# RichardZJM/lammps-mtp-kokkos

Hardware: AMD Instinct MI355X
Metric: atom-steps/s (64k-atom W, level-16 MTP) (higher is better)
Workload: dtype f64; 1 GPU; 65536-atom BCC W (a=3.165 A, +-0.05 A jitter, seed 777), W_L16.mtp (B=130 T=894 S=116 A=332 R=8 Mu=4 C=149), rc=5 A, full list 7 A, eflag=1 vflag=1; atoms=65536, potential=W_L16.mtp, parallelism=single GPU, atoms_rank0=65536, list_entries_rank0=5802796

## Files before the change

lammps_mtp_kokkos_amd/csrc/mtp_context.hip:

```cpp
#include <hip/hip_runtime.h>

#include <unistd.h>

#include <algorithm>
#include <cerrno>
#include <cmath>
#include <cstdio>
#include <cstdlib>
#include <cstring>
#include <new>
#include <string>
#include <vector>

#include "../../include/mtp_mi355x.h"
#include "mtp_device.hpp"
#include "mtp_shape_fields.hpp"
#include "mtp_potential.hpp"

namespace {

struct HipFail {
  hipError_t e;
  const char *what;
};
// ... 391 lines not shown
  bb.off_pack = put(pot.basic_pack_lds.data(), pot.basic_pack_lds.size() * sizeof(int32_t));
  blob.resize((blob.size() + 15) / 16 * 16, 0);
  bs.norows = (int) blob.size();
  bb.off_rows = put(rows8.data(), rows8.size() * sizeof(MtpRow8));
  bb.off_leaf_cf = put(pot.leaf_cf.data(), pot.leaf_cf.size() * sizeof(double));
  bb.off_leaf_cb = pot.leaf_cb == pot.leaf_cf ? bb.off_leaf_cf : put(pot.leaf_cb.data(), pot.leaf_cb.size() * sizeof(double));
  blob.resize((blob.size() + 15) / 16 * 16, 0);
  bs.rows = (int) blob.size();
  bb.blob_bytes = bs.norows;
  bb.rows_in_lds = 0;
}

void fill_sizes(const mtp_potential &pot, MtpDevParams &b)
{
  b.Sp = pot.species_count;
  b.R = pot.radial_basis_size;
  b.Mu = pot.radial_func_count;
  b.P = pot.max_alpha_index_basic;
  b.A = pot.alpha_moment_count;
  b.B = pot.alpha_index_basic_count;
  b.T = pot.alpha_index_times_count;
  b.S = pot.alpha_scalar_count;
  b.C = pot.coeff_count;
  b.nslot = pot.slot_count;
  b.coef_total = pot.coef_total;
  b.coef_dense = pot.coef_dense;
  for (int d = 0; d <= MTP_PSTRIDE; d++) {
    b.deg_first[d] = pot.deg_first[d];
    b.deg_coef[d] = pot.deg_coef[d];
  }
  b.nlevels = pot.normal_levels;
  const bool lv_fit = pot.level_offset.size() == (size_t) pot.normal_levels + 2 && pot.level_offset.size() <= MTP_SHAPE_ARR_LEN;
  for (int k = 0; k < MTP_SHAPE_ARR_LEN; k++) b.level_rows[k] = lv_fit && k < (int) pot.level_offset.size() ? pot.level_offset[k] : 0;
  b.nseed = (int) pot.seed_idx.size();
  b.Ad = pot.stored_moment_count;
  b.Am = b.Ad;
  b.Se = (int) pot.e_map.size();
}

void pad_and_tile(const double *W, int C, int cpad, std::vector<double> &pad, std::vector<double> &tiled)
{
  pad.assign((size_t) cpad * cpad, 0.0);
  for (int r = 0; r < C; r++) std::memcpy(&pad[(size_t) r * cpad], &W[(size_t) r * C], (size_t) C * sizeof(double));
  tiled.assign((size_t) cpad * cpad, 0.0);
  const int ks_n = cpad / 4;
  for (int t = 0; t < cpad / 16; t++)
    for (int ks = 0; ks < ks_n; ks++)
      for (int l = 0; l < 64; l++)
        tiled[((size_t) t * ks_n + ks) * 64 + l] = pad[(size_t) (16 * t + (l & 15)) * cpad + 4 * ks + (l >> 4)];
}

double cfg_grade_of(const double *W, int C, const double *c)
{
  double mx = 0.0;
  for (int i = 0; i < C; i++) {
    const double *row = &W[(size_t) i * C];
    double g = 0.0;
    for (int j = 0; j < C; j++) g += c[j] * row[j];
    mx = std::max(mx, g < 0 ? -g : g);
  }
  return mx;
}

bool all_finite(const double *v, size_t n)
{
  for (size_t i = 0; v && i < n; i++)
// ... 1698 lines not shown
}

extern "C" {

int mtp_plan_fixed_fields(const mtp_potential *pot, int num_cus, int inum, int max_numneigh, int variant, int grade,
                          char *buf, int buflen)
{
  MtpDevParams p;
  int rc = plan_params(pot, num_cus, inum, max_numneigh, variant, grade, p);
  if (rc != MTP_OK) return rc;
  if (!buf || buflen <= 0) return MTP_ERR_ARG;
  int KL = 0, NB = 0;
  (void) mtp_pick_fwd_shape(p.nfb, &KL, &NB);
  const int dlow = mtp_wave_kernel_deg(KL, p.P) == mtp_wave_kernel_dlow(KL);
  std::string s;
  auto put = [&](const char *k, int v) { s += std::string(k) + "=" + std::to_string(v) + "\n"; };
  put("KL", KL);
  put("NB", NB);
  put("PITCH", MTP_PITCH);
  put("GRADE", grade ? 1 : 0);
  put("DEG", mtp_wave_kernel_deg(KL, p.P));
  put("WPS", dlow && p.wps == 3 ? 3 : 2);
#define MTP_X(f) put(#f, p.f);
  MTP_SHAPE_INT_FIELDS(MTP_X)
#undef MTP_X
#define MTP_X(f)                                                                          \
  {                                                                                       \
    s += #f "=";                                                                          \
    for (int k = 0; k < MTP_SHAPE_ARR_LEN; k++) s += (k ? "," : "") + std::to_string(p.f[k]); \
    s += "\n";                                                                            \
  }
  MTP_SHAPE_ARR_FIELDS(MTP_X)
#undef MTP_X
  if ((int) s.size() + 1 > buflen) return MTP_ERR_LIMIT;
  std::memcpy(buf, s.c_str(), s.size() + 1);
  return MTP_OK;
}

int mtp_plan_fixed_shape(const mtp_potential *pot, int num_cus, int inum, int max_numneigh, int variant, int grade,
                         char *name, int namelen)
{
  MtpDevParams p;
  int rc = plan_params(pot, num_cus, inum, max_numneigh, variant, grade, p);
  if (rc != MTP_OK) return rc;
  if (!name || namelen <= 0) return MTP_ERR_ARG;
  const char *m = mtp_fixed_shape_match(p);
  std::snprintf(name, (size_t) namelen, "%s", m ? m : "");
  return MTP_OK;
}

int mtp_context_last_shape(const mtp_context *c, char *name, int namelen)
{
  if (!c || !name || namelen <= 0) return MTP_ERR_ARG;
  std::snprintf(name, (size_t) namelen, "%s", c->last_shape);
  return MTP_OK;
}

}

void *mtp_internal_resolve_stream(mtp_context *c, void *stream)
{
  return stream ? stream : (c ? reinterpret_cast<void *>(c->stream) : nullptr);
}

int mtp_internal_finish_unpack(mtp_context *c, void *stream, int eflag, int vflag, double *d_ev, double *d_f, const int *d_idx,
                               const double *d_frecv, int n3)
// ... 49 lines not shown
```

lammps_mtp_kokkos_amd/csrc/mtp_device.hpp:

```cpp
#pragma once

#include <hip/hip_runtime.h>

#include <cstddef>
#include <cstdint>

#define MTP_EV_SLOTS 4096
#define MTP_MAX_WPB 12
#define MTP_PITCH 33
#define MTP_PSTRIDE 12

struct alignas(8) MtpRow8 {
  uint32_t lo, hi;
};

struct MtpDevParams {
  int Sp, R, Mu, P, A, B, T, S, C;
  int nslot, nlevels, nseed;
  int Am, Ad, Se;
  const double *leaf_cf, *leaf_cb;
  const int *g_map_all;
  int deg_first[MTP_PSTRIDE + 2], deg_coef[MTP_PSTRIDE + 2];
  int level_rows[MTP_PSTRIDE + 2];
  int coef_total;
  int coef_dense;
  double rmin, rmax, scaling, cutsq, inv_span;
  double inv_rmax;
  const unsigned char *blob;
  int blob_bytes;
  int off_rows;
  int off_level;
  int off_slot;
  int off_radial;
  int off_seed_idx;
  int off_seed_val;
  int off_map;
  int off_lin;
  int off_pack;
  int off_fwd;
  int nfb;
  int off_smu;
  int off_coef;
  int off_leaf_cf, off_leaf_cb;
// ... 11 lines not shown
  const int *ilist, *first, *neigh;
  const double *x;
  const int *type;
  double *f;
  long long *fq;
  double *eatom;
  double *vatom;
  double *ev_slots;
  double *cvec;
  int cpad;
  double *dbasic;
  int dpad;
  int *err_flag;
  unsigned long long *stamps;
  int eflag, vflag, grade_flag;
  int xcd_map;
  int grade_fused;
  int NT;
  int tab_rows;
  int dg_mode;
  int fp_row;
  int rebuild_tables;
  int pow_row;
  int dg_off;
  int w_m, w_d, w_coef, w_nb;
  int wps;
  int row0;
  int ov_doubles;
  int cj_cap;
  int wave_doubles;
  int m_doubles;
  int d_doubles;
  float inv_mu;
};

int mtp_pick_shape(int B, int *KL, int *KB);
int mtp_pick_fwd_shape(int nblk, int *KL, int *NB);
constexpr int mtp_wave_kernel_dlow(int KL) { return KL <= 32 ? 6 : 8; }
constexpr int mtp_wave_kernel_deg(int KL, int P) { return P - 1 <= mtp_wave_kernel_dlow(KL) ? mtp_wave_kernel_dlow(KL) : 11; }
hipError_t mtp_launch_wave_kernel(const MtpDevParams &p, int grid, int wpb, size_t lds, hipStream_t st,
                                  const char **used = nullptr);
bool mtp_wave_kernel_has_wps3(int nfb, int P);
hipError_t mtp_launch_ev_finish(double *ev_slots, double *ev, hipStream_t st);
hipError_t mtp_launch_ev_finish_unpack(double *ev_slots, double *ev, int fold, double *f, const int *idx, const double *frecv,
                                       int n3, hipStream_t st);
struct mtp_context;
int mtp_internal_finish_unpack(mtp_context *c, void *stream, int eflag, int vflag, double *d_ev, double *d_f, const int *d_idx,
                               const double *d_frecv, int n3);
void *mtp_internal_resolve_stream(mtp_context *c, void *stream);
hipError_t mtp_launch_fixed_to_force(long long *fq, double *f, int nall, hipStream_t st);
hipError_t mtp_launch_zero(double *p, size_t n, hipStream_t st);
const char *mtp_kernel_build_flags();
hipError_t mtp_launch_cvec_kernel(const MtpDevParams &p, int grid, int wpb, size_t lds, hipStream_t st);
hipError_t mtp_launch_grade_kernel(const double *cvec, const double *ainv_pad, const double *ainv_tiled, int cpad,
                                   int C, int inum, const int *ilist, double *grades, double *max_grade, hipStream_t st);
hipError_t mtp_launch_colsum_kernel(const double *cvec, int cpad, int C, int inum, double *coeff_ders, hipStream_t st);
#define MTP_BATCH_BLOCK 256
#define MTP_BATCH_WAVE_ROWS 256
hipError_t mtp_launch_batch_reduce(int ncfg, const int *cfg_first, const double *eatom, const double *vatom, const double *grades,
                                   double *energy, double *virial, double *cfg_grade, hipStream_t st);
hipError_t mtp_launch_batch_colsum(const double *cvec, int cpad, int ncfg, const int *cfg_first, double *csum, int *ident,
                                   hipStream_t st);
hipError_t mtp_launch_batch_grade_scale(int ncfg, const int *cfg_first, double *cfg_grade, hipStream_t st);
const char *mtp_maxvol_build_flags();
size_t mtp_maxvol_arena_doubles(int num_cus, int C, long long N, int max_swaps);
hipError_t mtp_maxvol_run(hipStream_t st, int num_cus, double *arena, int C, const double *S, const double *W,
                          const double *d_rows, long long N, int ld, double threshold, int max_swaps, int refresh, double *S_out,
// ... 58 lines not shown
```

lammps_mtp_kokkos_amd/csrc/mtp_fixed_shapes.hpp:

```cpp
#pragma once

struct Shape_w16_force_3ps {
  static constexpr const char *name = "w16_force_3ps";
  static constexpr int kKL = 32;
  static constexpr int kNB = 1;
  static constexpr int kPITCH = 33;
  static constexpr bool kGRADE = false;
  static constexpr int kDEG = 6;
  static constexpr int kWPS = 3;
  static constexpr int Sp = 1;
  static constexpr int R = 8;
  static constexpr int Mu = 4;
  static constexpr int P = 7;
  static constexpr int A = 332;
  static constexpr int B = 130;
  static constexpr int T = 894;
  static constexpr int S = 116;
  static constexpr int C = 149;
  static constexpr int nslot = 16;
  static constexpr int nlevels = 3;
  static constexpr int nseed = 46;
  static constexpr int Am = 262;
  static constexpr int Ad = 262;
  static constexpr int Se = 46;
// ... 2 lines not shown
  static constexpr int coef_dense = 1;
  static constexpr int blob_bytes = 13888;
  static constexpr int off_rows = 4160;
  static constexpr int off_level = 0;
  static constexpr int off_slot = 128;
  static constexpr int off_radial = 320;
  static constexpr int off_seed_idx = 576;
  static constexpr int off_seed_val = 768;
  static constexpr int off_map = 1136;
  static constexpr int off_lin = 1328;
  static constexpr int off_pack = 3632;
  static constexpr int off_fwd = 1760;
  static constexpr int off_smu = 1696;
  static constexpr int off_coef = 2592;
  static constexpr int off_leaf_cf = 12352;
  static constexpr int off_leaf_cb = 12352;
  static constexpr int off_seg_fwd = 32;
  static constexpr int off_seg_bwd = 80;
  static constexpr int rows_in_lds = 1;
  static constexpr int tgt_in_lds = 1;
  static constexpr int scalars_in_lds = 1;
  static constexpr int dg_mode = 1;
  static constexpr int fp_row = 24;
  static constexpr int pow_row = 16;
  static constexpr int dg_off = 0;
  static constexpr int w_m = 528;
  static constexpr int w_d = 790;
  static constexpr int w_coef = 528;
  static constexpr int w_nb = 1221;
  static constexpr int tab_rows = 53;
  static constexpr int ov_doubles = 1221;
  static constexpr int m_doubles = 262;
  static constexpr int d_doubles = 262;
  static constexpr int deg_first(int k)
  {
    constexpr int v[14] = {0, 4, 7, 10, 12, 14, 15, 16, 16, 16, 16, 16, 16, 0};
    return v[k];
  }
  static constexpr int deg_coef(int k)
  {
    constexpr int v[14] = {0, 4, 13, 40, 76, 136, 181, 244, 244, 244, 244, 244, 244, 0};
    return v[k];
  }
  static constexpr int level_rows(int k)
  {
    constexpr int v[14] = {0, 640, 768, 832, 1024, 0, 0, 0, 0, 0, 0, 0, 0, 0};
    return v[k];
  }
};

struct Shape_w16_grade_3ps {
  static constexpr const char *name = "w16_grade_3ps";
  static constexpr int kKL = 32;
  static constexpr int kNB = 1;
  static constexpr int kPITCH = 33;
  static constexpr bool kGRADE = true;
  static constexpr int kDEG = 6;
  static constexpr int kWPS = 3;
  static constexpr int Sp = 1;
  static constexpr int R = 8;
  static constexpr int Mu = 4;
  static constexpr int P = 7;
  static constexpr int A = 332;
  static constexpr int B = 130;
  static constexpr int T = 894;
  static constexpr int S = 116;
  static constexpr int C = 149;
  static constexpr int nslot = 16;
  static constexpr int nlevels = 3;
  static constexpr int nseed = 46;
  static constexpr int Am = 332;
  static constexpr int Ad = 262;
  static constexpr int Se = 46;
  static constexpr int nfb = 26;
  static constexpr int coef_total = 244;
  static constexpr int coef_dense = 1;
  static constexpr int blob_bytes = 13888;
  static constexpr int off_rows = 4160;
  static constexpr int off_level = 0;
// ... 38 lines not shown
```

lammps_mtp_kokkos_amd/csrc/mtp_kernels.hip:

```cpp
#include <hip/hip_runtime.h>

#include <type_traits>

#include "mtp_device.hpp"

#include "mtp_kernel_common.hpp"
#include "mtp_wave_body.hpp"

namespace {

template <int KL, int NB, int PITCH, bool GRADE, int DEG, int WPS>
__global__ void __launch_bounds__(WPS == 3 ? 768 : 512, WPS) mtp_wave_kernel(const MtpDevParams p_arg)
{
  (void) p_arg;
  using SH = ShapeGeneric;
#include "mtp_wave_kernel_body.hpp"
}

__global__ void __launch_bounds__(256) mtp_fixed_to_force(long long *__restrict__ fq, double *__restrict__ f, int n3)
{
  const int e = blockIdx.x * 256 + threadIdx.x;
  if (e >= n3) return;
  const long long q = fq[e];
  if (q != 0) {
// ... 596 lines not shown

const char *mtp_kernel_build_flags()
{
#define MTP_STR2(x) #x
#define MTP_STR(x) MTP_STR2(x)
  return ""
#if MTP_PU != 2
      "MTP_PU=" MTP_STR(MTP_PU) " "
#endif
#if MTP_LD != 1
      "MTP_LD=" MTP_STR(MTP_LD) " "
#endif
#if MTP_POLY_CH != 8
      "MTP_POLY_CH=" MTP_STR(MTP_POLY_CH) " "
#endif
#if MTP_POLY_ACC != 1
      "MTP_POLY_ACC=" MTP_STR(MTP_POLY_ACC) " "
#endif
#if MTP_COEF_DPP != 1
      "MTP_COEF_DPP=" MTP_STR(MTP_COEF_DPP) " "
#endif
#if MTP_LEAF_SWEEP != 1
      "MTP_LEAF_SWEEP=" MTP_STR(MTP_LEAF_SWEEP) " "
#endif
#if MTP_E_HOIST != 1
      "MTP_E_HOIST=" MTP_STR(MTP_E_HOIST) " "
#endif
#if MTP_MU_BITS != 1
      "MTP_MU_BITS=" MTP_STR(MTP_MU_BITS) " "
#endif
#if MTP_LEVEL_ARGS != 1
      "MTP_LEVEL_ARGS=" MTP_STR(MTP_LEVEL_ARGS) " "
#endif

#if MTP_GRADE_TPB != 512 || MTP_GRADE_WPE != 2
      "MTP_GRADE_TPB=" MTP_STR(MTP_GRADE_TPB) " "
#endif
      ;
}

hipError_t mtp_launch_zero(double *p, size_t n, hipStream_t st)
{
  if (n == 0) return hipSuccess;
  const size_t n2 = n / 2;
  hipLaunchKernelGGL(mtp_zero_kernel, dim3((unsigned) ((std::max<size_t>(n2, 1) + 255) / 256)), dim3(256), 0, st,
                     reinterpret_cast<double2 *>(p), n2, p + 2 * n2, (int) (n - 2 * n2));
  return hipGetLastError();
}
```

lammps_mtp_kokkos_amd/csrc/mtp_shape_fields.hpp:

```cpp
#pragma once

#include <type_traits>

#include "mtp_device.hpp"

#define MTP_SHAPE_INT_FIELDS(X)                                                                                       \
  X(Sp) X(R) X(Mu) X(P) X(A) X(B) X(T) X(S) X(C) X(nslot) X(nlevels) X(nseed) X(Am) X(Ad) X(Se) X(nfb)                \
  X(coef_total) X(coef_dense) X(blob_bytes) X(off_rows) X(off_level) X(off_slot) X(off_radial) X(off_seed_idx)        \
  X(off_seed_val) X(off_map) X(off_lin) X(off_pack) X(off_fwd) X(off_smu) X(off_coef) X(off_leaf_cf) X(off_leaf_cb)   \
  X(off_seg_fwd) X(off_seg_bwd) X(rows_in_lds) X(tgt_in_lds) X(scalars_in_lds) X(dg_mode) X(fp_row) X(pow_row)        \
  X(dg_off) X(w_m) X(w_d) X(w_coef) X(w_nb) X(tab_rows) X(ov_doubles) X(m_doubles) X(d_doubles)
#define MTP_SHAPE_ARR_FIELDS(X) X(deg_first) X(deg_coef) X(level_rows)
#define MTP_SHAPE_ARR_LEN (MTP_PSTRIDE + 2)

struct ShapeGeneric {
  static constexpr const char *name = "";
};

namespace mtp_shape {

#define MTP_X(f)                                                                    \
  template <class SH, class = void> struct has_##f : std::false_type {};            \
  template <class SH> struct has_##f<SH, std::void_t<decltype(&SH::f)>> : std::true_type {};
MTP_SHAPE_INT_FIELDS(MTP_X)
MTP_SHAPE_ARR_FIELDS(MTP_X)
#undef MTP_X

template <class SH> bool matches(const MtpDevParams &p)
{
  bool ok = true;
#define MTP_X(f) \
  if constexpr (has_##f<SH>::value) ok = ok && p.f == SH::f;
  MTP_SHAPE_INT_FIELDS(MTP_X)
#undef MTP_X
#define MTP_X(f)                    \
  if constexpr (has_##f<SH>::value) \
    for (int k = 0; k < MTP_SHAPE_ARR_LEN; k++) ok = ok && p.f[k] == SH::f(k);
  MTP_SHAPE_ARR_FIELDS(MTP_X)
#undef MTP_X
  return ok;
}

}

const char *mtp_fixed_shape_match(const MtpDevParams &p);
hipError_t mtp_launch_wave_kernel_fixed(const MtpDevParams &p, int grid, int wpb, size_t lds, hipStream_t st, const char **used);
```

lammps_mtp_kokkos_amd/csrc/mtp_wave_body.hpp:

```cpp
#pragma once

#include <hip/hip_runtime.h>

#include <type_traits>

#include "mtp_device.hpp"

#include "mtp_kernel_common.hpp"
#include "mtp_shape_fields.hpp"

namespace {

#ifndef MTP_PU
#define MTP_PU 2
#endif

typedef const __attribute__((address_space(4))) MtpDevParams *KP;

namespace shape_get {
#define MTP_X(f)                                                                  \
  template <class SH> __device__ __forceinline__ int f(KP kp)                     \
  {                                                                               \
    if constexpr (mtp_shape::has_##f<SH>::value) return SH::f;                    \
    else return kp->f;                                                            \
  }
MTP_SHAPE_INT_FIELDS(MTP_X)
#undef MTP_X
#define MTP_X(f)                                                                  \
  template <class SH> __device__ __forceinline__ int f(KP kp, int k)              \
  {                                                                               \
    if constexpr (mtp_shape::has_##f<SH>::value) return SH::f(k);                 \
    else return kp->f[k];                                                         \
  }
MTP_SHAPE_ARR_FIELDS(MTP_X)
#undef MTP_X
}
#define SHF(f) (shape_get::f<SH>(kp))
#define SHA(f, k) (shape_get::f<SH>(kp, (k)))

#define MTP_FIXED_SCALE 1099511627776.0
static __device__ __forceinline__ void force_add(KP kp, size_t idx, double v)
{
  if (kp->fq) atomicAdd(reinterpret_cast<unsigned long long *>(kp->fq) + idx, (unsigned long long) __double2ll_rn(v * MTP_FIXED_SCALE));
  else unsafeAtomicAdd(&kp->f[idx], v);
}

template <int PITCH> struct WaveLds {
  static constexpr int NT = 32;
  double *M, *D, *coef, *tab, *nbx, *nby, *nbz, *nbr, *nbi;
  int *nbj, *nbjt, *cj;
  unsigned m_addr;
  __device__ __forceinline__ unsigned addr(const double *ptr) const { return m_addr + 8u * (unsigned) (ptr - M); }
  template <class SH> __device__ __forceinline__ WaveLds(double *base, unsigned base_addr, KP kp, SH)
  {
    tab = base;
    M = tab + SHF(w_m);
    D = tab + SHF(w_d);
    coef = tab + SHF(w_coef);
    nbx = tab + SHF(w_nb);
    m_addr = base_addr + 8u * (unsigned) (M - tab);
    nby = nbx + NT;
    nbz = nby + NT;
    nbr = nbz + NT;
    nbi = nbr + NT;
    nbj = reinterpret_cast<int *>(nbi + NT);
    nbjt = nbj + NT;
    cj = nbjt + NT;
  }
};

#define MTP_PARK 2
template <int PITCH, class SH>
__device__ __forceinline__ void build_tile(KP kp, const BlockTables &bt, const WaveLds<PITCH> &w,
                                           int t0, int cnt, int ntp, bool gather, bool powers, bool with_dg, bool do_park,
                                           double (&park)[MTP_PARK],
                                           double xi0, double xi1, double xi2, int i, int itype, int lane)
{
  if (gather) {
    if (lane < ntp) {
      const bool real = t0 + lane < cnt;
      const int j = real ? w.cj[t0 + lane] : i;
      double dx = 0, dy = 0, dz = 0, r = kp->rmax, inv = kp->inv_rmax;
      if (real) {
        const double *xj = row3(kp->x, j);
        dx = xj[0] - xi0;
        dy = xj[1] - xi1;
        dz = xj[2] - xi2;
        sqrt_and_inverse(dx * dx + dy * dy + dz * dz, r, inv);
      }
      w.nbx[lane] = dx;
      w.nby[lane] = dy;
      w.nbz[lane] = dz;
      w.nbr[lane] = r;
      w.nbi[lane] = inv;
      w.nbj[lane] = j;
      w.nbjt[lane] = real ? kp->type[j] - 1 : itype;
    }
    wave_fence();
  }
  const int Mu = SHF(Mu), P = SHF(P), R = SHF(R);
  const double mult = 2.0 * kp->inv_span;
  const int n = lane & 31, h = lane >> 5;
  if (n < ntp) {
    const double r = w.nbr[n], inv = w.nbi[n];
    const int jt = w.nbjt[n];
    const double d = r - kp->rmax;
    const double ksi = (2.0 * r - (kp->rmin + kp->rmax)) * kp->inv_span;
    double *col = w.tab + n;
    auto each_mu = [&](auto &&body) {
      double d0 = 0.0, d1 = 0.0;
      if (h < Mu) d0 = body(h);
      if (h + 2 < Mu) d1 = body(h + 2);
      for (int mu = h + 2 * MTP_PARK; mu < Mu; mu += 2) (void) body(mu);
      if (do_park) {
        park[0] = d0;
        park[1] = d1;
      }
    };
    if (R == 8) {
      double qv[8], ev[8];
      qv[0] = kp->scaling * (d * d);
      qv[1] = kp->scaling * (ksi * d * d);
      ev[0] = kp->scaling * 2.0 * d;
      ev[1] = kp->scaling * (mult * d * d + 2.0 * ksi * d);
#pragma unroll
      for (int ri = 2; ri < 8; ri++) {
        qv[ri] = 2.0 * ksi * qv[ri - 1] - qv[ri - 2];
        ev[ri] = 2.0 * (mult * qv[ri - 1] + ksi * ev[ri - 1]) - ev[ri - 2];
      }
      each_mu([&](int mu) {
        const int4 *sl4 = reinterpret_cast<const int4 *>(bt.slot + mu * MTP_PSTRIDE);
        const int4 sa = sl4[0], sb = sl4[1], sc = sl4[2];
        const int sv[MTP_PSTRIDE] = {sa.x, sa.y, sa.z, sa.w, sb.x, sb.y, sb.z, sb.w, sc.x, sc.y, sc.z, sc.w};
        const double2 *c2 = reinterpret_cast<const double2 *>(bt.radial + (mul24(itype * SHF(Sp) + jt, Mu) + mu) * 8);
        const double2 c01 = c2[0], c23 = c2[1], c45 = c2[2], c67 = c2[3];
        const double cc[8] = {c01.x, c01.y, c23.x, c23.y, c45.x, c45.y, c67.x, c67.y};
        double val = cc[0] * qv[0], der = cc[0] * ev[0];
#pragma unroll
        for (int ri = 1; ri < 8; ri++) {
          val = fma(cc[ri], qv[ri], val);
          der = fma(cc[ri], ev[ri], der);
        }
        double rp = 1.0;
#pragma unroll
        for (int nu = 0; nu < MTP_PSTRIDE; nu++) {
          if (nu < P) {
            const int sidx = sv[nu];
            const double g = val * rp;
            if (sidx >= 0) {
              double *gp = col + mul24(sidx, PITCH);
              *gp = g;
              if (with_dg) gp[SHF(dg_off)] = der * rp - nu * g * inv;
            }
            rp *= inv;
          }
        }
        return der;
      });
    } else {
      each_mu([&](int mu) {
        const int *sl = bt.slot + mu * MTP_PSTRIDE;
        const double *c = bt.radial + mul24(mul24(itype * SHF(Sp) + jt, Mu) + mu, R);
// ... 412 lines not shown
  constexpr int K = (C + 15) / 16;
  double c[K];
#pragma unroll
  for (int k = 0; k < K; k++) c[k] = lds_ld(coef_l, 16 * k);
  double a = 0.0;
  dpp_chunks<C, 0>(a, c, m);
  return a;
}
template <int C> constexpr bool coef_dpp = MTP_COEF_DPP && C >= 2;
template <int C> __device__ __forceinline__ double poly_sum(unsigned coef, const double *m)
{
  if constexpr (coef_dpp<C>) return poly_eval_dpp<C>(coef, m);
  else return poly_eval<C>(coef, m);
}

#ifndef MTP_MU_BITS
#define MTP_MU_BITS 1
#endif
template <bool PACKED> struct SlotMu {
  const int *smu;
  unsigned long long bits;
  template <bool NODG, bool GRADE> __device__ __forceinline__ int uniform(int s) const
  {
    if constexpr (PACKED) return (int) (bits >> (2 * s)) & 3;
    else return (NODG || GRADE) ? __builtin_amdgcn_readfirstlane(smu[s]) : 0;
  }
  template <bool NODG, bool GRADE> __device__ __forceinline__ int per_lane(int s) const
  {
    if constexpr (PACKED) return (int) (bits >> (2 * s)) & 3;
    else return (NODG || GRADE) ? smu[s] : 0;
  }
};

template <int NU, int DEG, int PITCH, bool GRADE, bool NODG, class SH, class SMU>
__device__ __forceinline__ void force_degree(KP kp, unsigned pcol, unsigned pcoef, unsigned pcoef_l, int part, double x,
                                             double y, double z, double *m, double &UA, double &VA, double &UB,
                                             double &VB, const SMU &smu, double inv, double rw, double *W)
{
  if constexpr (NU <= DEG) {
    constexpr int C = NU * (NU + 1) / 2;
    const unsigned pc = coef_dpp<C> ? pcoef_l : pcoef;
    if (NU < SHF(P)) {
      const int s0 = SHA(deg_first, NU), cnt = SHA(deg_first, NU + 1) - s0;
      const double inv_nu = 1.0 / NU;
      const unsigned dgo = 8u * (unsigned) SHF(dg_off);
      const unsigned pfp = pcol + 8u * (unsigned) (SHF(fp_row) * PITCH);
      const double rwn = rw * inv_nu;
      const double wa = GRADE ? (part ? z : x) * rwn : 0.0, wb = GRADE ? y * rwn : 0.0;
      {
        unsigned ca = pc + 8u * (unsigned) (SHA(deg_coef, NU) + part * 2 * C);
        unsigned cg = pcol + 8u * (unsigned) (s0 * PITCH);
        for (int it = 0; it < cnt; it++) {
          const int mu = smu.template uniform<NODG, GRADE>(s0 + it);
          const double g = lds_ld(cg, 0);
          const double dg = NODG ? lds_ld(pfp + 8u * (unsigned) (mu * PITCH), 0) : lds_ld(cg + dgo, 0);
          const double G = poly_sum<C>(ca, m);
          UA = fma(g, G, UA);
          VA = fma(dg * (NODG ? rwn : inv_nu), G, VA);
          if (GRADE) {
            const double val = G * wa;
            if (mu == 0) W[0] += val;
            else if (mu == 1) W[1] += val;
            else if (mu == 2) W[2] += val;
            else W[3] += val;
          }
          ca += 8u * 3 * C;
          cg += 8u * PITCH;
        }
      }
      for (int it = 0; 2 * it < cnt; it++) {
        const int si = 2 * it + part;
        const bool ok = si < cnt;
        const int sc = ok ? si : 0;
        const unsigned cb = pc + 8u * (unsigned) (SHA(deg_coef, NU) + C) + (unsigned) mul24(sc, 8 * 3 * C);
        const unsigned cg = pcol + (unsigned) mul24(s0 + sc, 8 * PITCH);
        const int mu_raw = smu.template per_lane<NODG, GRADE>(s0 + sc);
        const double g_raw = lds_ld(cg, 0);
        const double dg_raw = NODG ? lds_ld(pfp + (unsigned) mul24(mu_raw, 8 * PITCH), 0) : lds_ld(cg + dgo, 0);
        const double G = poly_sum<C>(cb, m);
        const double g = ok ? g_raw : 0.0, dg = ok ? dg_raw : 0.0;
        UB = fma(g, G, UB);
        VB = fma(dg * (NODG ? rwn : inv_nu), G, VB);
        const int mu = ok ? mu_raw : -1;
        if (GRADE) {
          const double val = G * wb;
#pragma unroll
          for (int v = 0; v < 4; v++) W[v] += mu == v ? val : 0.0;
        }
      }
      if constexpr (NU < DEG) {
        constexpr int T0 = (NU - 1) * NU / 2;
#pragma unroll
        for (int c = 0; c < NU; c++) m[C + c] = y * m[T0 + c];
        m[C + NU] = z * m[T0 + NU - 1];
#pragma unroll
        for (int i = 0; i < C; i++) m[i] *= x;
        force_degree<NU + 1, DEG, PITCH, GRADE, NODG, SH>(kp, pcol, pcoef, pcoef_l, part, x, y, z, m, UA, VA, UB, VB, smu, inv, rw * inv, W);
      }
    }
  }
}

}
```

lammps_mtp_kokkos_amd/csrc/mtp_wave_kernel_body.hpp:

```cpp
  constexpr int NT = 32;
  constexpr bool GATHER = KL == 64;
  constexpr bool NODG_CT = WPS == 3;
  constexpr int NG = 64 / KL;
  constexpr int NPG = NT / NG;
  static_assert(NT == 32, "the force phase maps lanes to (32 neighbours) x (2 halves)");

  KP kp = (KP) __builtin_amdgcn_kernarg_segment_ptr();
#ifdef MTP_STAMPS
  const unsigned long long st_entry = __builtin_amdgcn_s_memtime();
#endif
  kernarg_touch<(int) sizeof(MtpDevParams)>(kp);
  extern __shared__ double lds[];
  unsigned char *sh = reinterpret_cast<unsigned char *>(lds);
  const int lane = threadIdx.x & 63;
  const int wave = __builtin_amdgcn_readfirstlane(threadIdx.x >> 6);
  const int wpb = blockDim.x >> 6;

  int ii_beg, ii_end, ii_step;
  if (kp->xcd_map && (gridDim.x & 7) == 0) {
    const int chunk = (kp->inum + 7) >> 3, xcd = blockIdx.x & 7;
    const int nb8 = gridDim.x >> 3;
    if (chunk % (nb8 * wpb) != 0) ii_beg = kp->row0 + xcd * chunk + wave * nb8 + (blockIdx.x >> 3);
    else ii_beg = kp->row0 + xcd * chunk + (blockIdx.x >> 3) * wpb + wave;
    ii_end = kp->row0 + min(kp->inum, (xcd + 1) * chunk);
    ii_step = (gridDim.x >> 3) * wpb;
  } else {
    ii_step = gridDim.x * wpb;
    if (kp->inum % ii_step != 0) ii_beg = kp->row0 + wave * gridDim.x + blockIdx.x;
    else ii_beg = kp->row0 + blockIdx.x * wpb + wave;
    ii_end = kp->row0 + kp->inum;
  }
  int hd_i = 0, hd_b = 0, hd_e = 0;
  if (ii_beg < ii_end) {
    hd_i = kp->ilist[ii_beg];
    hd_b = kp->first[ii_beg];
    hd_e = kp->first[ii_beg + 1];
  }
  for (int o = threadIdx.x * 16; o < SHF(blob_bytes); o += blockDim.x * 16)
    *reinterpret_cast<uint4 *>(sh + o) = *reinterpret_cast<const uint4 *>(kp->blob + o);
  __syncthreads();
  BlockTables bt;
  bt.rows = reinterpret_cast<const MtpRow8 *>(sh + SHF(off_rows));
  bt.level = reinterpret_cast<const int *>(sh + SHF(off_level));
  bt.seg_fwd = reinterpret_cast<const int *>(sh + SHF(off_seg_fwd));
  bt.seg_bwd = reinterpret_cast<const int *>(sh + SHF(off_seg_bwd));
  bt.slot = reinterpret_cast<const int *>(sh + SHF(off_slot));
  bt.radial = reinterpret_cast<const double *>(sh + SHF(off_radial));
  bt.seed_idx = reinterpret_cast<const int *>(sh + SHF(off_seed_idx));
  bt.seed_val = reinterpret_cast<const double *>(sh + SHF(off_seed_val));
  bt.map = reinterpret_cast<const int *>(sh + SHF(off_map));
  bt.lin = reinterpret_cast<const double *>(sh + SHF(off_lin));
  bt.pack = reinterpret_cast<const int *>(sh + SHF(off_pack));
  bt.coef = reinterpret_cast<const int *>(sh + SHF(off_coef));
  bt.smu = reinterpret_cast<const int *>(sh + SHF(off_smu));
  bt.fwd = reinterpret_cast<const int *>(sh + SHF(off_fwd));
  bt.leaf_cf = reinterpret_cast<const double *>(sh + SHF(off_leaf_cf));
  bt.leaf_cb = reinterpret_cast<const double *>(sh + SHF(off_leaf_cb));
  const bool rows_lds = SHF(rows_in_lds) != 0;
  constexpr bool MU_PACKED = MTP_MU_BITS && WPS == 3 && !(GRADE && KL == 16);
  SlotMu<MU_PACKED> smu{bt.smu, 0ull};
  if constexpr (MU_PACKED) {
    const int mu_l = lane < min(SHF(nslot), 32) ? bt.smu[lane] : 0;
    const unsigned long long b0 = __ballot((mu_l & 1) != 0), b1 = __ballot((mu_l & 2) != 0);
    auto spread = [](unsigned long long x) {
      x = (x | (x << 16)) & 0x0000ffff0000ffffull;
      x = (x | (x << 8)) & 0x00ff00ff00ff00ffull;
      x = (x | (x << 4)) & 0x0f0f0f0f0f0f0f0full;
      x = (x | (x << 2)) & 0x3333333333333333ull;
      return (x | (x << 1)) & 0x5555555555555555ull;
    };
    smu.bits = spread(b0) | (spread(b1) << 1);
  }

  const int kl = lane & (KL - 1), q = lane / KL;
  const unsigned wave_off = (SHF(blob_bytes) >> 3) + wave * kp->wave_doubles;
  const unsigned lds0 = (unsigned) (size_t) (lds_cdouble *) lds;
  const WaveLds<PITCH> w(lds + wave_off, lds0 + 8u * wave_off, kp, SH{});
  const int P = SHF(P);

  unsigned hg[NB][3], hx[NB][3], ty[NB][3], tz[NB][3];
  bool bval[NB];
  auto block_addresses = [&](int kl_) {
#pragma unroll
    for (int t = 0; t < NB; t++) {
      const int blk = kl_ + KL * t;
      bval[t] = blk < SHF(nfb);
      const int *bd = bt.fwd + 8 * (bval[t] ? blk : 0);
      const unsigned w0 = (unsigned) bd[0], w1 = (unsigned) bd[1], w2 = (unsigned) bd[2];
#pragma unroll
      for (int h = 0; h < 3; h++) {
        const unsigned tq = w.addr(w.tab + q);
        hg[t][h] = tq + (unsigned) mul24((int) ((w0 >> (8 * h)) & 255u), 8 * PITCH);
        hx[t][h] = tq + (unsigned) mul24(SHF(pow_row) + (int) ((w1 >> (4 * h)) & 15u), 8 * PITCH);
        ty[t][h] = tq + (unsigned) mul24(SHF(pow_row) + P + (int) ((w1 >> (12 + 4 * h)) & 15u), 8 * PITCH);
// ... 274 lines not shown
#pragma unroll
        for (int u = 0; u < ROUNDS; u++) tg[u] = reinterpret_cast<const int2 *>(bt.coef)[min(k0 + lane + 64 * u, SHF(B) - 1)];
      } else {
#pragma unroll
        for (int u = 0; u < ROUNDS; u++) tg[u] = reinterpret_cast<const int2 *>(kp->g_tgt)[min(k0 + lane + 64 * u, SHF(B) - 1)];
      }
#pragma unroll
      for (int u = 0; u < ROUNDS; u++) dd[u] = w.D[min(k0 + lane + 64 * u, SHF(B) - 1)];
#pragma unroll
      for (int u = 0; u < ROUNDS; u++) {
        const int k = k0 + lane + 64 * u;
        const bool ok = k < SHF(B);
        if (GRADE && kp->dbasic && k < kp->dpad) kp->dbasic[(size_t) ii * kp->dpad + k] = ok ? dd[u] : 0.0;
        if (ok) {
          const unsigned t0 = (unsigned) tg[u].x, t1 = (unsigned) tg[u].y;
          const unsigned tx = t0 & 0xffffu, ty_ = t0 >> 16, tz_ = t1 & 0xffffu;
          if (tx != 0xffffu) w.coef[tx] = dd[u] * (double) ((t1 >> 16) & 15u);
          if (ty_ != 0xffffu) w.coef[ty_] = dd[u] * (double) ((t1 >> 20) & 15u);
          if (tz_ != 0xffffu) w.coef[tz_] = dd[u] * (double) ((t1 >> 24) & 15u);
        }
      }
    }
    wave_fence();
    STAMP(9);
    {
      const int n = lane & 31, part = lane >> 5;
      unsigned pcol = w.addr(w.tab + n);
      asm volatile("" : "+v"(pcol));
      double crad = 0.0;
      for (int tile = 0; tile < ntiles; tile++) {
        const int t0 = tile * NT, nt = min(NT, cnt - t0), ntp = ((nt + NG - 1) / NG) * NG;
        if (ntiles > 1 || rebuild)
          build_tile<PITCH, SH>(kp, bt, w, t0, cnt, ntp, ntiles > 1, false, !nodg, nodg, park, xi0, xi1, xi2, i, itype, lane);
        if (nodg) fp_from_parked<PITCH, SH>(kp, w, ntp, park, lane);
        const double x = w.nbx[n], y = w.nby[n], z = w.nbz[n], inv = w.nbi[n];
        double UA = 0.0, VA = 0.0, UB = 0.0, VB = 0.0, S0 = 0.0;
        double Wm[4] = {0.0, 0.0, 0.0, 0.0};
        const bool fused = GRADE && kp->grade_fused;
        const unsigned pcoef = w.addr(w.coef), pcoef_l = pcoef + 8u * (unsigned) (lane & 15);
        {
          const unsigned cg0 = pcol + 8u * (unsigned) (nodg ? SHF(fp_row) * PITCH : SHF(dg_off));
          const int n0 = SHA(deg_first, 1);
#if MTP_COEF_DPP
          for (int s4 = 0; s4 < n0; s4 += 4) {
            const double c = lds_ld(pcoef_l + 8u * (unsigned) (SHA(deg_coef, 0) + s4), 0);
            auto term = [&](auto I) {
              constexpr int i = decltype(I)::value;
              const int sidx = s4 + i;
              if (i == 0 || sidx < n0) {
                const int mu = nodg ? smu.template uniform<true, GRADE>(sidx) : smu.template uniform<false, GRADE>(sidx);
                fmac_row_bcast1<i>(S0, c, lds_ld(cg0 + 8u * (unsigned) ((nodg ? mu : sidx) * PITCH), 0));
                if (GRADE) {
                  const double dk = row_bcast<i>(c);
#pragma unroll
                  for (int v = 0; v < 4; v++) Wm[v] += (mu == v && part == 0) ? dk : 0.0;
                }
              }
            };
            term(std::integral_constant<int, 0>());
            term(std::integral_constant<int, 1>());
            term(std::integral_constant<int, 2>());
            term(std::integral_constant<int, 3>());
          }
#else
          for (int sidx = 0; sidx < n0; sidx++) {
            const double dk = w.coef[SHA(deg_coef, 0) + sidx];
            const int mu = nodg ? smu.template uniform<true, GRADE>(sidx) : smu.template uniform<false, GRADE>(sidx);
            S0 = fma(lds_ld(cg0 + 8u * (unsigned) ((nodg ? mu : sidx) * PITCH), 0), dk, S0);
            if (GRADE) {
#pragma unroll
              for (int v = 0; v < 4; v++) Wm[v] += (mu == v && part == 0) ? dk : 0.0;
            }
          }
#endif
        }
        double mono[DEG * (DEG + 1) / 2];
        mono[0] = 1.0;
        if (nodg) {
          force_degree<1, DEG, PITCH, GRADE, true, SH>(kp, pcol, pcoef, pcoef_l, part, x, y, z, mono, UA, VA, UB, VB, smu, inv, inv, Wm);
          VA = fma(-inv, UA, VA);
          VB = fma(-inv, UB, VB);
        } else if constexpr (!NODG_CT) {
          force_degree<1, DEG, PITCH, GRADE, false, SH>(kp, pcol, pcoef, pcoef_l, part, x, y, z, mono, UA, VA, UB, VB, smu, inv, inv, Wm);
        }
        if (fused) {
          double qv[8];
          {
            const double r = w.nbr[n], d = r - kp->rmax;
            const double ksi = (2.0 * r - (kp->rmin + kp->rmax)) * kp->inv_span;
            qv[0] = kp->scaling * (d * d);
            qv[1] = kp->scaling * (ksi * d * d);
#pragma unroll
            for (int ri = 2; ri < 8; ri++) qv[ri] = 2.0 * ksi * qv[ri - 1] - qv[ri - 2];
          }
          const bool mine = n < nt && w.nbjt[n] == part;
          double ent[32];
#pragma unroll
          for (int v = 0; v < 4; v++) {
            const double wt = pair_sum32(Wm[v]);
#pragma unroll
            for (int ri = 0; ri < 8; ri++) ent[8 * v + ri] = mine ? qv[ri] * wt : 0.0;
          }
          Butterfly<32>::run(ent, lane);
          crad += ent[0];
        }
        double S = fma(y, VB, (part ? z : x) * VA) + (part ? 0.0 : S0);
        S = pair_sum32(S);
        UB = pair_sum32(UB);
        const double sr = S * inv;
        const bool valid = n < nt;
        const double Fa = valid ? fma(sr, part ? z : x, UA) : 0.0;
        const double Fy = valid && part == 0 ? fma(sr, y, UB) : 0.0;
        const double Fx = part ? 0.0 : Fa, Fz = part ? Fa : 0.0;
        if (valid) {
          const size_t j = (size_t) w.nbj[n];
          unsigned j2 = (unsigned) j << 1;
// ... 84 lines not shown
```

Before: 193.1 million atom-steps/s.

## Bake slot-row and slot-mu tables into fixed shapes; keep radial derivatives in registers

Adds compile-time slot_row and packed slot_mu tables to the fixed-shape specialization. The radial basis build can then scatter values to constant LDS rows without loading the slot table, and the SlotMu bits become a constant with no ballot needed. In the nodg path, the parked radial derivatives are swapped across wave halves with permlane32_swap and selected from registers instead of being written to and re-read from LDS. This removes LDS traffic and table loads in exchange for more code specialization and possibly higher register pressure.

After: 200.7 million atom-steps/s, median of 6. +4.0%, better.

```diff
diff --git a/lammps_mtp_kokkos_amd/csrc/mtp_context.hip b/lammps_mtp_kokkos_amd/csrc/mtp_context.hip
--- a/lammps_mtp_kokkos_amd/csrc/mtp_context.hip
+++ b/lammps_mtp_kokkos_amd/csrc/mtp_context.hip
@@ -447,6 +447,17 @@
   b.nlevels = pot.normal_levels;
   const bool lv_fit = pot.level_offset.size() == (size_t) pot.normal_levels + 2 && pot.level_offset.size() <= MTP_SHAPE_ARR_LEN;
   for (int k = 0; k < MTP_SHAPE_ARR_LEN; k++) b.level_rows[k] = lv_fit && k < (int) pot.level_offset.size() ? pot.level_offset[k] : 0;
+  unsigned long long mu_bits = 0;
+  if (pot.radial_func_count <= 4 && pot.slot_count <= 32)
+    for (int s = 0; s < pot.slot_count; s++) mu_bits |= (unsigned long long) (pot.slot_mu[s] & 3) << (2 * s);
+  b.slot_mu_lo = (int) (unsigned) mu_bits;
+  b.slot_mu_hi = (int) (unsigned) (mu_bits >> 32);
+  const bool sr_fit = pot.radial_func_count <= MTP_SLOT_ROWS_MU && pot.slot_count <= 127 && pot.max_alpha_index_basic <= MTP_PSTRIDE;
+  for (int k = 0; k < MTP_SHAPE_TAB_LEN; k++) {
+    const int mu = k / MTP_PSTRIDE, nu = k % MTP_PSTRIDE;
+    const bool in = sr_fit && mu < pot.radial_func_count && nu < pot.max_alpha_index_basic;
+    b.slot_row[k] = (signed char) (in ? pot.slot_of[(size_t) mu * pot.max_alpha_index_basic + nu] : -1);
+  }
   b.nseed = (int) pot.seed_idx.size();
   b.Ad = pot.stored_moment_count;
   b.Am = b.Ad;
@@ -2211,6 +2222,14 @@
   }
   MTP_SHAPE_ARR_FIELDS(MTP_X)
 #undef MTP_X
+#define MTP_X(f)                                                                               \
+  {                                                                                            \
+    s += #f "=";                                                                               \
+    for (int k = 0; k < MTP_SHAPE_TAB_LEN; k++) s += (k ? "," : "") + std::to_string((int) p.f[k]); \
+    s += "\n";                                                                                 \
+  }
+  MTP_SHAPE_TAB_FIELDS(MTP_X)
+#undef MTP_X
   if ((int) s.size() + 1 > buflen) return MTP_ERR_LIMIT;
   std::memcpy(buf, s.c_str(), s.size() + 1);
   return MTP_OK;
diff --git a/lammps_mtp_kokkos_amd/csrc/mtp_device.hpp b/lammps_mtp_kokkos_amd/csrc/mtp_device.hpp
--- a/lammps_mtp_kokkos_amd/csrc/mtp_device.hpp
+++ b/lammps_mtp_kokkos_amd/csrc/mtp_device.hpp
@@ -9,6 +9,7 @@
 #define MTP_MAX_WPB 12
 #define MTP_PITCH 33
 #define MTP_PSTRIDE 12
+#define MTP_SLOT_ROWS_MU 4
 
 struct alignas(8) MtpRow8 {
   uint32_t lo, hi;
@@ -86,7 +87,10 @@
   int m_doubles;
   int d_doubles;
   float inv_mu;
+  int slot_mu_lo, slot_mu_hi;
+  signed char slot_row[MTP_SLOT_ROWS_MU * MTP_PSTRIDE];
 };
+static_assert(sizeof(MtpDevParams) <= 12 * 64, "the force kernel's argument block: twelve 64-byte lines (kernarg_touch)");
 
 int mtp_pick_shape(int B, int *KL, int *KB);
 int mtp_pick_fwd_shape(int nblk, int *KL, int *NB);
diff --git a/lammps_mtp_kokkos_amd/csrc/mtp_fixed_shapes.hpp b/lammps_mtp_kokkos_amd/csrc/mtp_fixed_shapes.hpp
--- a/lammps_mtp_kokkos_amd/csrc/mtp_fixed_shapes.hpp
+++ b/lammps_mtp_kokkos_amd/csrc/mtp_fixed_shapes.hpp
@@ -58,6 +58,8 @@
   static constexpr int ov_doubles = 1221;
   static constexpr int m_doubles = 262;
   static constexpr int d_doubles = 262;
+  static constexpr int slot_mu_lo = 71902436;
+  static constexpr int slot_mu_hi = 0;
   static constexpr int deg_first(int k)
   {
     constexpr int v[14] = {0, 4, 7, 10, 12, 14, 15, 16, 16, 16, 16, 16, 16, 0};
@@ -71,6 +73,11 @@
   static constexpr int level_rows(int k)
   {
     constexpr int v[14] = {0, 640, 768, 832, 1024, 0, 0, 0, 0, 0, 0, 0, 0, 0};
+    return v[k];
+  }
+  static constexpr int slot_row(int k)
+  {
+    constexpr int v[48] = {0, 4, 7, 10, 12, 14, 15, -1, -1, -1, -1, -1, 1, 5, 8, 11, 13, -1, -1, -1, -1, -1, -1, -1, 2, 6, 9, -1, -1, -1, -1, -1, -1, -1, -1, -1, 3, -1, -1, -1, -1, -1, -1, -1, -1, -1, -1, -1};
     return v[k];
   }
 };
diff --git a/lammps_mtp_kokkos_amd/csrc/mtp_kernels.hip b/lammps_mtp_kokkos_amd/csrc/mtp_kernels.hip
--- a/lammps_mtp_kokkos_amd/csrc/mtp_kernels.hip
+++ b/lammps_mtp_kokkos_amd/csrc/mtp_kernels.hip
@@ -652,6 +652,12 @@
 #if MTP_LEVEL_ARGS != 1
       "MTP_LEVEL_ARGS=" MTP_STR(MTP_LEVEL_ARGS) " "
 #endif
+#if MTP_SLOT_ARGS != 1
+      "MTP_SLOT_ARGS=" MTP_STR(MTP_SLOT_ARGS) " "
+#endif
+#if MTP_FP_REGS != 1
+      "MTP_FP_REGS=" MTP_STR(MTP_FP_REGS) " "
+#endif
 
 #if MTP_GRADE_TPB != 512 || MTP_GRADE_WPE != 2
       "MTP_GRADE_TPB=" MTP_STR(MTP_GRADE_TPB) " "
diff --git a/lammps_mtp_kokkos_amd/csrc/mtp_shape_fields.hpp b/lammps_mtp_kokkos_amd/csrc/mtp_shape_fields.hpp
--- a/lammps_mtp_kokkos_amd/csrc/mtp_shape_fields.hpp
+++ b/lammps_mtp_kokkos_amd/csrc/mtp_shape_fields.hpp
@@ -9,9 +9,12 @@
   X(coef_total) X(coef_dense) X(blob_bytes) X(off_rows) X(off_level) X(off_slot) X(off_radial) X(off_seed_idx)        \
   X(off_seed_val) X(off_map) X(off_lin) X(off_pack) X(off_fwd) X(off_smu) X(off_coef) X(off_leaf_cf) X(off_leaf_cb)   \
   X(off_seg_fwd) X(off_seg_bwd) X(rows_in_lds) X(tgt_in_lds) X(scalars_in_lds) X(dg_mode) X(fp_row) X(pow_row)        \
-  X(dg_off) X(w_m) X(w_d) X(w_coef) X(w_nb) X(tab_rows) X(ov_doubles) X(m_doubles) X(d_doubles)
+  X(dg_off) X(w_m) X(w_d) X(w_coef) X(w_nb) X(tab_rows) X(ov_doubles) X(m_doubles) X(d_doubles)                     \
+  X(slot_mu_lo) X(slot_mu_hi)
 #define MTP_SHAPE_ARR_FIELDS(X) X(deg_first) X(deg_coef) X(level_rows)
 #define MTP_SHAPE_ARR_LEN (MTP_PSTRIDE + 2)
+#define MTP_SHAPE_TAB_FIELDS(X) X(slot_row)
+#define MTP_SHAPE_TAB_LEN (MTP_SLOT_ROWS_MU * MTP_PSTRIDE)
 
 struct ShapeGeneric {
   static constexpr const char *name = "";
@@ -24,6 +27,7 @@
   template <class SH> struct has_##f<SH, std::void_t<decltype(&SH::f)>> : std::true_type {};
 MTP_SHAPE_INT_FIELDS(MTP_X)
 MTP_SHAPE_ARR_FIELDS(MTP_X)
+MTP_SHAPE_TAB_FIELDS(MTP_X)
 #undef MTP_X
 
 template <class SH> bool matches(const MtpDevParams &p)
@@ -38,6 +42,11 @@
     for (int k = 0; k < MTP_SHAPE_ARR_LEN; k++) ok = ok && p.f[k] == SH::f(k);
   MTP_SHAPE_ARR_FIELDS(MTP_X)
 #undef MTP_X
+#define MTP_X(f)                    \
+  if constexpr (has_##f<SH>::value) \
+    for (int k = 0; k < MTP_SHAPE_TAB_LEN; k++) ok = ok && p.f[k] == SH::f(k);
+  MTP_SHAPE_TAB_FIELDS(MTP_X)
+#undef MTP_X
   return ok;
 }
 
diff --git a/lammps_mtp_kokkos_amd/csrc/mtp_wave_body.hpp b/lammps_mtp_kokkos_amd/csrc/mtp_wave_body.hpp
--- a/lammps_mtp_kokkos_amd/csrc/mtp_wave_body.hpp
+++ b/lammps_mtp_kokkos_amd/csrc/mtp_wave_body.hpp
@@ -3,6 +3,7 @@
 #include <hip/hip_runtime.h>
 
 #include <type_traits>
+#include <utility>
 
 #include "mtp_device.hpp"
 
@@ -33,10 +34,56 @@
     else return kp->f[k];                                                         \
   }
 MTP_SHAPE_ARR_FIELDS(MTP_X)
+MTP_SHAPE_TAB_FIELDS(MTP_X)
 #undef MTP_X
 }
 #define SHF(f) (shape_get::f<SH>(kp))
 #define SHA(f, k) (shape_get::f<SH>(kp, (k)))
+#define SHT(f, k) (shape_get::f<SH>(kp, (k)))
+
+template <class F, int... I> __device__ __forceinline__ void static_for(F &&f, std::integer_sequence<int, I...>)
+{
+  (f(std::integral_constant<int, I>()), ...);
+}
+
+#ifndef MTP_SLOT_ARGS
+#define MTP_SLOT_ARGS 1
+#endif
+template <class SH>
+constexpr bool slot_rows_ct = MTP_SLOT_ARGS && mtp_shape::has_slot_row<SH>::value && mtp_shape::has_Mu<SH>::value &&
+    mtp_shape::has_P<SH>::value && mtp_shape::has_R<SH>::value;
+template <class SH>
+constexpr bool slot_mu_shape = mtp_shape::has_slot_mu_lo<SH>::value && mtp_shape::has_slot_mu_hi<SH>::value &&
+    mtp_shape::has_nslot<SH>::value && mtp_shape::has_Mu<SH>::value;
+template <class SH> constexpr bool slot_mu_ct = MTP_SLOT_ARGS && slot_mu_shape<SH>;
+template <class SH> constexpr unsigned long long slot_mu_bits()
+{
+  if constexpr (slot_mu_shape<SH>) return ((unsigned long long) (unsigned) SH::slot_mu_hi << 32) | (unsigned) SH::slot_mu_lo;
+  else return 0ull;
+}
+template <class SH> __device__ __forceinline__ int slot_mu_of(int s) { return (int) (slot_mu_bits<SH>() >> (2 * s)) & 3; }
+#ifndef MTP_FP_REGS
+#define MTP_FP_REGS 1
+#endif
+template <class SH>
+constexpr bool fp_regs_ct = MTP_FP_REGS && slot_mu_shape<SH> && mtp_shape::has_deg_first<SH>::value;
+#define MTP_FP_N 4
+__device__ __forceinline__ void fp_exchange(const double (&park)[2], double (&F)[MTP_FP_N])
+{
+#pragma unroll
+  for (int mi = 0; mi < 2; mi++) {
+    const long long b = __double_as_longlong(park[mi]);
+    const unsigned lo = (unsigned) b, hi = (unsigned) (b >> 32);
+    const auto a = __builtin_amdgcn_permlane32_swap(lo, lo, false, false);
+    const auto c = __builtin_amdgcn_permlane32_swap(hi, hi, false, false);
+    F[2 * mi] = __longlong_as_double((long long) (((unsigned long long) c[0] << 32) | a[0]));
+    F[2 * mi + 1] = __longlong_as_double((long long) (((unsigned long long) c[1] << 32) | a[1]));
+  }
+}
+__device__ __forceinline__ double fp_pick(const double (&F)[MTP_FP_N], int mu)
+{
+  return mu == 0 ? F[0] : mu == 1 ? F[1] : mu == 2 ? F[2] : F[3];
+}
 
 #define MTP_FIXED_SCALE 1099511627776.0
 static __device__ __forceinline__ void force_add(KP kp, size_t idx, double v)
@@ -70,6 +117,15 @@
 };
 
 #define MTP_PARK 2
+template <class SH, int MI> constexpr int slot_delta()
+{
+  if (2 * MI + 1 < SH::Mu)
+    for (int nu = 0; nu < SH::P; nu++) {
+      const int r0 = SH::slot_row(2 * MI * MTP_PSTRIDE + nu), r1 = SH::slot_row((2 * MI + 1) * MTP_PSTRIDE + nu);
+      if (r0 >= 0 && r1 >= 0) return r1 - r0;
+    }
+  return 0;
+}
 template <int PITCH, class SH>
 __device__ __forceinline__ void build_tile(KP kp, const BlockTables &bt, const WaveLds<PITCH> &w,
                                            int t0, int cnt, int ntp, bool gather, bool powers, bool with_dg, bool do_park,
@@ -128,6 +184,54 @@
         qv[ri] = 2.0 * ksi * qv[ri - 1] - qv[ri - 2];
         ev[ri] = 2.0 * (mult * qv[ri - 1] + ksi * ev[ri - 1]) - ev[ri - 2];
       }
+      if constexpr (slot_rows_ct<SH>) {
+        static_assert(SH::Mu <= 2 * MTP_PARK && SH::Mu <= MTP_SLOT_ROWS_MU && SH::P <= MTP_PSTRIDE && SH::R == 8, "slot_row: the nodg tables");
+        double dpark[MTP_PARK] = {0.0, 0.0};
+        static_for([&](auto MI) {
+          constexpr int mi = decltype(MI)::value, mu0 = 2 * mi, mu1 = 2 * mi + 1;
+          if constexpr (mu0 < SH::Mu) {
+            constexpr bool two = mu1 < SH::Mu;
+            const int mu = two ? mu0 + h : mu0;
+            if (two || h == 0) {
+              const double2 *c2 = reinterpret_cast<const double2 *>(bt.radial + (mul24(itype * SHF(Sp) + jt, Mu) + mu) * 8);
+              const double2 c01 = c2[0], c23 = c2[1], c45 = c2[2], c67 = c2[3];
+              const double cc[8] = {c01.x, c01.y, c23.x, c23.y, c45.x, c45.y, c67.x, c67.y};
+              double val = cc[0] * qv[0], der = cc[0] * ev[0];
+#pragma unroll
+              for (int ri = 1; ri < 8; ri++) {
+                val = fma(cc[ri], qv[ri], val);
+                der = fma(cc[ri], ev[ri], der);
+              }
+              constexpr int delta = slot_delta<SH, mi>();
+              double *colh = col + (h ? delta * PITCH : 0);
+              double rp = 1.0;
+              static_for([&](auto NU) {
+                constexpr int nu = decltype(NU)::value;
+                constexpr int r0 = SH::slot_row(mu0 * MTP_PSTRIDE + nu), r1 = two ? SH::slot_row(mu1 * MTP_PSTRIDE + nu) : -1;
+                const double g = val * rp;
+                auto put = [&](double *gp) {
+                  *gp = g;
+                  if (with_dg) gp[SHF(dg_off)] = der * rp - nu * g * inv;
+                };
+                if constexpr (r0 >= 0 && r1 >= 0) {
+                  if constexpr (r1 - r0 == delta) put(colh + r0 * PITCH);
+                  else put(col + (h ? r1 * PITCH : r0 * PITCH));
+                } else if constexpr (r0 >= 0) {
+                  if (h == 0) put(col + r0 * PITCH);
+                } else if constexpr (r1 >= 0) {
+                  if (h == 1) put(col + r1 * PITCH);
+                }
+                rp *= inv;
+              }, std::make_integer_sequence<int, SH::P>());
+              dpark[mi] = der;
+            }
+          }
+        }, std::make_integer_sequence<int, MTP_PARK>());
+        if (do_park) {
+          park[0] = dpark[0];
+          park[1] = dpark[1];
+        }
+      } else
       each_mu([&](int mu) {
         const int4 *sl4 = reinterpret_cast<const int4 *>(bt.slot + mu * MTP_PSTRIDE);
         const int4 sa = sl4[0], sb = sl4[1], sc = sl4[2];
@@ -606,10 +710,11 @@
   }
 };
 
-template <int NU, int DEG, int PITCH, bool GRADE, bool NODG, class SH, class SMU>
+template <int NU, int DEG, int PITCH, bool GRADE, bool NODG, class SH, class SMU, bool FPR = false>
 __device__ __forceinline__ void force_degree(KP kp, unsigned pcol, unsigned pcoef, unsigned pcoef_l, int part, double x,
                                              double y, double z, double *m, double &UA, double &VA, double &UB,
-                                             double &VB, const SMU &smu, double inv, double rw, double *W)
+                                             double &VB, const SMU &smu, double inv, double rw, double *W,
+                                             const double (&F)[MTP_FP_N])
 {
   if constexpr (NU <= DEG) {
     constexpr int C = NU * (NU + 1) / 2;
@@ -627,7 +732,9 @@
         for (int it = 0; it < cnt; it++) {
           const int mu = smu.template uniform<NODG, GRADE>(s0 + it);
           const double g = lds_ld(cg, 0);
-          const double dg = NODG ? lds_ld(pfp + 8u * (unsigned) (mu * PITCH), 0) : lds_ld(cg + dgo, 0);
+          double dg;
+          if constexpr (FPR) dg = fp_pick(F, slot_mu_of<SH>(s0 + it));
+          else dg = NODG ? lds_ld(pfp + 8u * (unsigned) (mu * PITCH), 0) : lds_ld(cg + dgo, 0);
           const double G = poly_sum<C>(ca, m);
           UA = fma(g, G, UA);
           VA = fma(dg * (NODG ? rwn : inv_nu), G, VA);
@@ -650,7 +757,14 @@
         const unsigned cg = pcol + (unsigned) mul24(s0 + sc, 8 * PITCH);
         const int mu_raw = smu.template per_lane<NODG, GRADE>(s0 + sc);
         const double g_raw = lds_ld(cg, 0);
-        const double dg_raw = NODG ? lds_ld(pfp + (unsigned) mul24(mu_raw, 8 * PITCH), 0) : lds_ld(cg + dgo, 0);
+        double dg_raw;
+        if constexpr (FPR) {
+          const double f0 = fp_pick(F, slot_mu_of<SH>(s0 + 2 * it));
+          const double f1 = 2 * it + 1 < cnt ? fp_pick(F, slot_mu_of<SH>(s0 + 2 * it + 1)) : 0.0;
+          dg_raw = part ? f1 : f0;
+        } else {
+          dg_raw = NODG ? lds_ld(pfp + (unsigned) mul24(mu_raw, 8 * PITCH), 0) : lds_ld(cg + dgo, 0);
+        }
         const double G = poly_sum<C>(cb, m);
         const double g = ok ? g_raw : 0.0, dg = ok ? dg_raw : 0.0;
         UB = fma(g, G, UB);
@@ -669,10 +783,10 @@
         m[C + NU] = z * m[T0 + NU - 1];
 #pragma unroll
         for (int i = 0; i < C; i++) m[i] *= x;
-        force_degree<NU + 1, DEG, PITCH, GRADE, NODG, SH>(kp, pcol, pcoef, pcoef_l, part, x, y, z, m, UA, VA, UB, VB, smu, inv, rw * inv, W);
-      }
-    }
-  }
-}
-
-}
+        force_degree<NU + 1, DEG, PITCH, GRADE, NODG, SH, SMU, FPR>(kp, pcol, pcoef, pcoef_l, part, x, y, z, m, UA, VA, UB, VB, smu, inv, rw * inv, W, F);
+      }
+    }
+  }
+}
+
+}
diff --git a/lammps_mtp_kokkos_amd/csrc/mtp_wave_kernel_body.hpp b/lammps_mtp_kokkos_amd/csrc/mtp_wave_kernel_body.hpp
--- a/lammps_mtp_kokkos_amd/csrc/mtp_wave_kernel_body.hpp
+++ b/lammps_mtp_kokkos_amd/csrc/mtp_wave_kernel_body.hpp
@@ -1,6 +1,7 @@
   constexpr int NT = 32;
   constexpr bool GATHER = KL == 64;
   constexpr bool NODG_CT = WPS == 3;
+  constexpr bool FP_REGS = NODG_CT && MTP_MU_BITS && fp_regs_ct<SH>;
   constexpr int NG = 64 / KL;
   constexpr int NPG = NT / NG;
   static_assert(NT == 32, "the force phase maps lanes to (32 neighbours) x (2 halves)");
@@ -59,7 +60,9 @@
   const bool rows_lds = SHF(rows_in_lds) != 0;
   constexpr bool MU_PACKED = MTP_MU_BITS && WPS == 3 && !(GRADE && KL == 16);
   SlotMu<MU_PACKED> smu{bt.smu, 0ull};
-  if constexpr (MU_PACKED) {
+  if constexpr (MU_PACKED && slot_mu_ct<SH>) {
+    smu.bits = slot_mu_bits<SH>();
+  } else if constexpr (MU_PACKED) {
     const int mu_l = lane < min(SHF(nslot), 32) ? bt.smu[lane] : 0;
     const unsigned long long b0 = __ballot((mu_l & 1) != 0), b1 = __ballot((mu_l & 2) != 0);
     auto spread = [](unsigned long long x) {
@@ -400,7 +403,9 @@
         const int t0 = tile * NT, nt = min(NT, cnt - t0), ntp = ((nt + NG - 1) / NG) * NG;
         if (ntiles > 1 || rebuild)
           build_tile<PITCH, SH>(kp, bt, w, t0, cnt, ntp, ntiles > 1, false, !nodg, nodg, park, xi0, xi1, xi2, i, itype, lane);
-        if (nodg) fp_from_parked<PITCH, SH>(kp, w, ntp, park, lane);
+        double Fp[MTP_FP_N] = {0.0, 0.0, 0.0, 0.0};
+        if constexpr (FP_REGS) fp_exchange(park, Fp);
+        else if (nodg) fp_from_parked<PITCH, SH>(kp, w, ntp, park, lane);
         const double x = w.nbx[n], y = w.nby[n], z = w.nbz[n], inv = w.nbi[n];
         double UA = 0.0, VA = 0.0, UB = 0.0, VB = 0.0, S0 = 0.0;
         double Wm[4] = {0.0, 0.0, 0.0, 0.0};
@@ -417,7 +422,8 @@
               const int sidx = s4 + i;
               if (i == 0 || sidx < n0) {
                 const int mu = nodg ? smu.template uniform<true, GRADE>(sidx) : smu.template uniform<false, GRADE>(sidx);
-                fmac_row_bcast1<i>(S0, c, lds_ld(cg0 + 8u * (unsigned) ((nodg ? mu : sidx) * PITCH), 0));
+                if constexpr (FP_REGS) fmac_row_bcast1<i>(S0, c, fp_pick(Fp, slot_mu_of<SH>(sidx)));
+                else fmac_row_bcast1<i>(S0, c, lds_ld(cg0 + 8u * (unsigned) ((nodg ? mu : sidx) * PITCH), 0));
                 if (GRADE) {
                   const double dk = row_bcast<i>(c);
 #pragma unroll
@@ -434,7 +440,8 @@
           for (int sidx = 0; sidx < n0; sidx++) {
             const double dk = w.coef[SHA(deg_coef, 0) + sidx];
             const int mu = nodg ? smu.template uniform<true, GRADE>(sidx) : smu.template uniform<false, GRADE>(sidx);
-            S0 = fma(lds_ld(cg0 + 8u * (unsigned) ((nodg ? mu : sidx) * PITCH), 0), dk, S0);
+            if constexpr (FP_REGS) S0 = fma(fp_pick(Fp, slot_mu_of<SH>(sidx)), dk, S0);
+            else S0 = fma(lds_ld(cg0 + 8u * (unsigned) ((nodg ? mu : sidx) * PITCH), 0), dk, S0);
             if (GRADE) {
 #pragma unroll
               for (int v = 0; v < 4; v++) Wm[v] += (mu == v && part == 0) ? dk : 0.0;
@@ -445,11 +452,11 @@
         double mono[DEG * (DEG + 1) / 2];
         mono[0] = 1.0;
         if (nodg) {
-          force_degree<1, DEG, PITCH, GRADE, true, SH>(kp, pcol, pcoef, pcoef_l, part, x, y, z, mono, UA, VA, UB, VB, smu, inv, inv, Wm);
+          force_degree<1, DEG, PITCH, GRADE, true, SH, SlotMu<MU_PACKED>, FP_REGS>(kp, pcol, pcoef, pcoef_l, part, x, y, z, mono, UA, VA, UB, VB, smu, inv, inv, Wm, Fp);
           VA = fma(-inv, UA, VA);
           VB = fma(-inv, UB, VB);
         } else if constexpr (!NODG_CT) {
-          force_degree<1, DEG, PITCH, GRADE, false, SH>(kp, pcol, pcoef, pcoef_l, part, x, y, z, mono, UA, VA, UB, VB, smu, inv, inv, Wm);
+          force_degree<1, DEG, PITCH, GRADE, false, SH>(kp, pcol, pcoef, pcoef_l, part, x, y, z, mono, UA, VA, UB, VB, smu, inv, inv, Wm, Fp);
         }
         if (fused) {
           double qv[8];
```
